# yeyupiaoling/PPASR

Hardware: AMD Instinct MI355X
Metric: audio-seconds/s (RTF^-1) Conformer-streaming fbank, batch32 per GPU, ctc_greedy (higher is better)
Workload: dtype f32; 1 GPU; configs[1]: Conformer streaming (configs/conformer.yml), fbank-80, 32 x 10 s utterances per GPU, V=4233, ctc_greedy, features resident in HBM -> token ids + scores on device; global_batch=32, frames=1000, decoder=ctc_greedy, parallelism=utterance-dp1, pipelined=False, gemm=f32

## Files before the change

ppasr_amd/csrc/capi.hip:

```cpp
#include <cxxabi.h>
#include <cstdlib>

#include "capi_internal.h"

namespace ppasr {
thread_local LaunchProf g_launch_prof;
}

static thread_local std::string g_err;
std::string& ppasr_err_slot() { return g_err; }


ppasr_status upload_pe_table(ppasr_model_s* m, BlobMap& sd, const float** pe_dev) {
  const int d = m->desc.output_size > 0 ? m->desc.output_size : kD;
  const int max_len = m->desc.max_len > 0 ? m->desc.max_len : 5000;
  m->desc.max_len = max_len;
  std::vector<float> pe((size_t)max_len * d);
  auto it = sd.find("__pe_table__");
  if (it != sd.end() && it->second.numel() == pe.size()) {
    std::memcpy(pe.data(), it->second.p, pe.size() * sizeof(float));
  } else {
    for (int i = 0; i < d / 2; ++i) {
      float div = expf((float)(2 * i) * (float)(-(std::log(10000.0) / d)));
      for (int pos = 0; pos < max_len; ++pos) {
// ... 166 lines not shown
    m->front.conv2_w = nullptr;
  } else {
    GET(mean, "encoder.global_cmvn.mean", F);
    GET(istd, "encoder.global_cmvn.istd", F);
    GET(c1w, "encoder.embed.conv.0.weight", d * 9);
    GET(c1b, "encoder.embed.conv.0.bias", d);
    const int k2 = il == 6 ? 5 : 3;
    GET(c2w, "encoder.embed.conv.2.weight", (size_t)d * d * k2 * k2);
    GET(c2b, "encoder.embed.conv.2.bias", d);
    const std::string lin = il ? "encoder.embed.linear" : "encoder.embed.out.0";
    GET(ew, lin + ".weight", (size_t)d * F2 * d);
    GET(eb, lin + ".bias", d);
    UP(vec_of(mean, F), m->front.cmvn_mean);
    UP(vec_of(istd, F), m->front.cmvn_istd);
    std::vector<float> c1(9 * d);
    for (int c = 0; c < d; ++c)
      for (int j = 0; j < 9; ++j) c1[j * d + c] = c1w[c * 9 + j];
    UP(c1, m->front.conv1_w);
    UP(vec_of(c1b, d), m->front.conv1_b);
    const int taps2 = k2 * k2;
    auto c2 = [&](int k, int n) { return c2w[((size_t)n * d + (k % d)) * taps2 + (k / d)]; };
    UP4(pack_b(taps2 * d, d, c2), m->front.conv2_w);
    m->front.conv2_wp = nullptr;
    if (il == 0 && d == kD) UP4(pack_conv2_pair(d, c2), m->front.conv2_wp);
    UP(vec_of(c2b, d), m->front.conv2_b);
    m->front.conv2_k = k2;
    m->front.conv2_s = il == 6 ? 3 : 2;
    m->front.conv3_w = nullptr;
    m->front.conv3_b = nullptr;
    if (il == 8) {
      GET(c3w, "encoder.embed.conv.4.weight", (size_t)d * d * 9);
      GET(c3b, "encoder.embed.conv.4.bias", d);
      UP4(pack_b(9 * d, d, [&](int k, int n) { return c3w[((size_t)n * d + (k % d)) * 9 + (k / d)]; }), m->front.conv3_w);
      UP(vec_of(c3b, d), m->front.conv3_b);
    }
    UP4(pack_b(F2 * d, d, [&](int k, int n) { return ew[((size_t)(k % d) * F2 + (k / d)) * d + n]; }), m->front.embed_w);
    UP(vec_of(eb, d), m->front.embed_b);
  }

  const float* pe_dev = nullptr;
  if ((st = upload_pe_table(m, sd, &pe_dev)) != PPASR_OK) return st;
  m->pe_dev = pe_dev;
  UP(std::vector<float>(d, 0.f), m->zero_vec);
  if (generic) m->gen_x.resize(desc->num_blocks);
  const int max_len = m->desc.max_len;
  m->layers.resize(desc->num_blocks);
  m->layer_ks.assign(desc->num_blocks, KS);
// ... 534 lines not shown
    PadSkip ps;
    if (skip) {
      ps.lens = lens;
      ps.Tp = Tcur;
      ps.mul = mul_cur;
      ps.slack = mul_cur == sub ? slack_full : slack_half;
    }
    return ps;
  };
  const f32x4* conv2_h3 = h->gemm_mode == PPASR_GEMM_F16X3 ? h->conv2_w_h3 : nullptr;
  const bool conv12 = h->desc.input_layer == 0 && !conv2_h3 && conv12_enabled(h) && conv12_supported(h->front, F, F2);
  const PadSkip ps_front = skip_front ? pskip(Tp, sub) : PadSkip{};
  if (!conv12) timed(0, [&] { launch_conv1(feats, h->front, y1, B, T, F, T1, F1, st, ps_front); });
  if (h->desc.input_layer == 8) {
    timed(1, [&] {
      launch_conv_stage(y1, h->front.conv2_w, h->front.conv2_b, y2, B, T1, F1, fd.T2, F2, 3, 2, st);
      launch_conv_stage(y2, h->front.conv3_w, h->front.conv3_b, y1, B, fd.T2, F2, Tp, h->F3, 3, 2, st);
    });
    timed(2, [&] { launch_embed(y1, h->front, xa, M, h->F3 * kD, sqrtf((float)kD), false, st, PadSkip{}, ffn_split_for(h, M), y2); });
  } else {
    timed(1, [&] {
      int* tile_tab = (size_t)B + 2 <= ((size_t)M + 63) / 64 * 64 ? reinterpret_cast<int*>(ws + wl.rmax) : nullptr;
      if (conv12) launch_conv12(feats, h->front, y2, B, T, F, Tp, F2, st, ps_front, tile_tab);
      else if (h->desc.input_layer == 0 && !conv2_h3 && conv2_pair_supported(h->front))
        launch_conv2_pair(y1, h->front, y2, B, T1, F1, Tp, F2, st, ps_front, tile_tab);
      else launch_conv2(y1, h->front, y2, B, T1, F1, Tp, F2, st, ps_front, tile_tab, h->desc.input_layer == 0 ? conv2_h3 : nullptr);
    });
    timed(2, [&] {
      launch_embed(y2, h->front, xa, M, F2 * kD, sqrtf((float)kD), false, st, ps_front, wide_slices_for(h, M, F2), y1,
                   conv2_h3 ? h->embed_w_h3 : nullptr);
    });
  }
  tap(xa, (size_t)M * kD);
  const int n_chunks = h->desc.linear_units / 256;
  struct BlkTab { int Ti, R; int* tab; } btabs[4];
  int n_bt = 0;
  size_t bt_off = ((size_t)B + 2 + 15) / 16 * 16;
  const bool bt_ok = skip && block_tables_enabled() && (size_t)B + 2 <= ((size_t)M + 63) / 64 * 64;
  auto with_table = [&](PadSkip p, int Tcur, int R) {
    if (!bt_ok) return p;
    for (int k = 0; k < n_bt; ++k)
      if (btabs[k].Ti == Tcur && btabs[k].R == R) { p.tab = btabs[k].tab; return p; }
    const size_t n = 1 + ((size_t)B * Tcur + R - 1) / R;
    if (n_bt == 4 || bt_off + n > 2 * (((size_t)M + 63) / 64 * 64)) return p;
    int* t = reinterpret_cast<int*>(ws + wl.rmax) + bt_off;
    launch_block_table(p, B * Tcur, R, t, st);
    btabs[n_bt++] = BlkTab{Tcur, R, t};
    bt_off += (n + 15) / 16 * 16;
// ... 767 lines not shown
```

ppasr_amd/csrc/capi_internal.h:

```cpp
#pragma once
#include <hip/hip_runtime.h>

#include <cmath>
#include <cstdio>
#include <cstring>
#include <memory>
#include <string>
#include <unordered_map>
#include <vector>

#include "../../include/ppasr_hip.h"
#include "conformer_kernels.h"
#include "launch.h"
#include "ctc_beam.h"

using namespace ppasr;

#include "squeezeformer_kernels.h"
#include "ds2_kernels.h"

std::string& ppasr_err_slot();
inline ppasr_status fail(ppasr_status s, const std::string& msg) {
  ppasr_err_slot() = msg;
  return s;
// ... 11 lines not shown
  size_t numel() const {
    size_t n = 1;
    for (int i = 0; i < ndim; ++i) n *= (size_t)shape[i];
    return n;
  }
};

template <typename Acc>
inline std::vector<float> pack_b(int K, int N, Acc w) {
  const int n_tiles = (N + 31) / 32, G = K / 8;
  std::vector<float> out((size_t)n_tiles * G * 256, 0.f);
  for (int nt = 0; nt < n_tiles; ++nt)
    for (int g = 0; g < G; ++g)
      for (int l = 0; l < 64; ++l) {
        int n = nt * 32 + (l & 31);
        if (n >= N) continue;
        float* dst = &out[(((size_t)nt * G + g) * 64 + l) * 4];
        for (int j = 0; j < 4; ++j) dst[j] = w(8 * g + 4 * (l >> 5) + j, n);
      }
  return out;
}

template <typename Acc>
inline std::vector<float> pack_conv2_pair(int d, Acc w) {
  return pack_b(24 * 128, d, [&](int k, int n) {
    const int s = k / 512, slab = (k / 128) & 3, kw = s >> 1, c = (s & 1) * 128 + (k & 127);
    const float g0 = w(kw * d + c, n), w1 = w((3 + kw) * d + c, n), g1 = w((6 + kw) * d + c, n);
    return slab == 0 ? g0 : slab == 1 ? w1 : slab == 2 ? g0 + g1 : g1;
  });
}

typedef std::unordered_map<std::string, Blob> BlobMap;

inline unsigned eff_stride_mask(const ppasr_model_desc& d) {
  if (d.model_type != PPASR_MODEL_EFFICIENT_CONFORMER) return 0u;
  if (d.stride_layer_mask != 0) return (unsigned)d.stride_layer_mask;
  return d.stride_layer_idx >= 0 ? (1u << d.stride_layer_idx) : 0u;
}
inline int eff_strides_before(const ppasr_model_desc& d, int layer) {
  return __builtin_popcount(eff_stride_mask(d) & ((1u << layer) - 1u));
}

struct ppasr_model_s {
  ppasr_model_desc desc;
  int F1, F2;
  const f32x4* gen_head_w = nullptr;
  const float* gen_head_b = nullptr;
  int gen_vpad = 0;
  int F3 = 0;
  struct Front {
    int T1, T2, Tp;
// ... 162 lines not shown
```

ppasr_amd/csrc/capi_squeezeformer.hip:

```cpp
#include "capi_internal.h"

namespace {

struct Getter {
  BlobMap& sd;
  std::string missing;
  const float* operator()(const std::string& name, size_t numel) {
    auto it = sd.find(name);
    if (it == sd.end() || it->second.numel() != numel) {
      if (missing.empty()) missing = name;
      return nullptr;
    }
    return it->second.p;
  }
};

std::vector<float> vec_of(const float* p, size_t n) { return std::vector<float>(p, p + n); }

}

#define GETW(var, name, numel)                 \
  const float* var = get(name, (size_t)(numel)); \
  if (!var) return fail(PPASR_EMISSING, "missing or mis-shaped weight: " + get.missing)
#define UP(vec, dst) \
// ... 26 lines not shown
    const bool dw_stride = !c2w;
    if (!c2w) {
      get.missing.clear();
      c2w = get("encoder.embed.dw_conv.weight", (size_t)d * 9);
    }
    if (!c2w) return fail(PPASR_EMISSING, "missing or mis-shaped weight: " + get.missing);
    GETW(c2b, "encoder.embed.dw_conv.bias", d);
    GETW(ew, "encoder.embed.input_proj.0.weight", (size_t)d * F2 * d);
    GETW(eb, "encoder.embed.input_proj.0.bias", d);
    GETW(pg, "encoder.preln.weight", d);
    GETW(pb, "encoder.preln.bias", d);
    UP(vec_of(mean, F), m->front.cmvn_mean);
    UP(vec_of(istd, F), m->front.cmvn_istd);
    std::vector<float> c1(9 * d);
    for (int c = 0; c < d; ++c)
      for (int j = 0; j < 9; ++j) c1[j * d + c] = c1w[c * 9 + j];
    UP(c1, m->front.conv1_w);
    UP(vec_of(c1b, d), m->front.conv1_b);
    auto c2 = [&](int k, int n) {
      if (dw_stride) return (k % d) == n ? c2w[(size_t)n * 9 + (k / d)] : 0.f;
      return c2w[((size_t)n * d + (k % d)) * 9 + (k / d)];
    };
    UP4(pack_b(9 * d, d, c2), m->front.conv2_w);
    if (d == kD) UP4(pack_conv2_pair(d, c2), m->front.conv2_wp);
    UP(vec_of(c2b, d), m->front.conv2_b);
    UP4(pack_b(F2 * d, d, [&](int k, int n) { return ew[((size_t)(k % d) * F2 + (k / d)) * d + n]; }), m->front.embed_w);
    UP(vec_of(eb, d), m->front.embed_b);
    UP(vec_of(pg, d), m->preln_g);
    UP(vec_of(pb, d), m->preln_b);
  }
  m->sq_layers.resize(L);
  for (int i = 0; i < L; ++i) {
    SqLayerW& W = m->sq_layers[i];
    const std::string p = "encoder.encoders." + std::to_string(i) + ".";
    auto ln = [&](const std::string& n, const float** g, const float** b) -> ppasr_status {
      const float* gw = get(p + n + ".weight", d);
      const float* gb = get(p + n + ".bias", d);
      if (!gw || !gb) return fail(PPASR_EMISSING, "missing or mis-shaped weight: " + get.missing);
      ppasr_status s1 = m->upload(vec_of(gw, d), g);
      return s1 != PPASR_OK ? s1 : m->upload(vec_of(gb, d), b);
    };
    if ((st = ln("layer_norm1", &W.ln1_g, &W.ln1_b)) != PPASR_OK) return st;
    if ((st = ln("layer_norm2", &W.ln2_g, &W.ln2_b)) != PPASR_OK) return st;
    if ((st = ln("layer_norm3", &W.ln3_g, &W.ln3_b)) != PPASR_OK) return st;
    if ((st = ln("layer_norm4", &W.ln4_g, &W.ln4_b)) != PPASR_OK) return st;
    W.cm_eps = 1e-5f;
    if (sd.find(p + "conv_module.norm._mean") != sd.end()) {
// ... 240 lines not shown
  };
  const PadSkip psF = pskip(Tp, 4), psH = pskip(Tr, 8);
  int* tile_tab = (size_t)B + 2 <= ((size_t)M + 63) / 64 * 64 ? reinterpret_cast<int*>(ws + wl.rmax) : nullptr;
  const int rowsF = h->taps ? 32 : row_block_for(h, B, Tp, 4, psF.slack, skip);
  const int rowsH = h->taps ? 32 : row_block_for(h, B, Tr, 8, psH.slack, skip);
  PadSkip psF_rb = psF, psH_rb = psH;
  if (skip && tile_tab && block_tables_enabled()) {
    const int RF = rowsF == 16 ? 16 : 32, RH = rowsH == 16 ? 16 : 32;
    const size_t nF = 1 + ((size_t)M + RF - 1) / RF, nH = 1 + ((size_t)B * Tr + RH - 1) / RH;
    const size_t o1 = ((size_t)B + 2 + 15) / 16 * 16, o2 = o1 + (nF + 15) / 16 * 16;
    if (o2 + nH <= 2 * (((size_t)M + 63) / 64 * 64)) {
      int* base = reinterpret_cast<int*>(ws + wl.rmax);
      launch_block_table(psF, M, RF, base + o1, st);
      launch_block_table(psH, B * Tr, RH, base + o2, st);
      psF_rb.tab = base + o1;
      psH_rb.tab = base + o2;
    }
  }
  const f32x4* conv2_h3 = h->gemm_mode == PPASR_GEMM_F16X3 ? h->conv2_w_h3 : nullptr;
  if (!conv2_h3 && conv12_enabled(h) && conv12_supported(h->front, F, F2)) {
    launch_conv12(feats, h->front, y2, B, T, F, Tp, F2, st, psF, tile_tab);
  } else {
    launch_conv1(feats, h->front, y1, B, T, F, T1, F1, st, psF);
    if (!conv2_h3 && conv2_pair_supported(h->front)) launch_conv2_pair(y1, h->front, y2, B, T1, F1, Tp, F2, st, psF, tile_tab);
    else launch_conv2(y1, h->front, y2, B, T1, F1, Tp, F2, st, psF, tile_tab, conv2_h3);
  }
  launch_embed(y2, h->front, xa, M, F2 * kD, sqrtf((float)kD), true, st,
               (rowsF != 16 && ffn_split_for(h, M) == 1) ? psF_rb : psF, ffn_split_for(h, M), y1,
               conv2_h3 ? h->embed_w_h3 : nullptr);
  launch_ln_rows(xa, h->preln_g, h->preln_b, M, st, psF);
  tap(xa, (size_t)M * kD);
  float* x = xa;
  float* other = xb;
  bool reduced = false;
  bool have_qkv = false;
  for (int i = 0; i < L; ++i) {
    const SqLayerW& W = h->sq_layers[i];
    if (i == h->desc.reduce_idx) {
      HIP_TRY(hipMemcpyAsync(xs, x, (size_t)M * kD * sizeof(float), hipMemcpyDeviceToDevice, st));
      launch_sq_reduce(x, other, qkv, h->sq_reduce, W.wqkv, W.bqkv, lens, B, Tp, Tr, st, psH);
      std::swap(x, other);
      reduced = true;
      have_qkv = true;
    }
    if (i == h->desc.recover_idx && reduced) {
      launch_sq_recover(x, xs, other, qkv, h->sq_wrec, h->sq_brec, W.wqkv, W.bqkv, B, Tp, Tr, st, psF);
      std::swap(x, other);
// ... 87 lines not shown
```

ppasr_amd/csrc/conformer_kernels.h:

```cpp
#pragma once
#include <hip/hip_runtime.h>
#include <stdint.h>

#include "rowblock.h"

namespace ppasr {

struct LayerW {
  const float *ln_mac_g, *ln_mac_b, *ln_mha_g, *ln_mha_b, *ln_conv_g, *ln_conv_b;
  const float *ln_ff_g, *ln_ff_b, *ln_fin_g, *ln_fin_b, *ln_cm_g, *ln_cm_b;
  float cm_eps;
  const f32x4 *ffm_w1, *ffm_w2, *ff_w1, *ff_w2, *wqkv, *wo, *pw1, *pw2;
  const float *ffm_b1, *ffm_b2, *ff_b1, *ff_b2, *bqkv, *bo, *pw1_b, *pw2_b;
  const float *dw_w;
  const float *dw_b;
  const float *glu_pad;
  const float *pos_u, *pos_v;
  const float *ptab;
};

struct FrontW {
  const float *cmvn_mean, *cmvn_istd;
  const float *conv1_w, *conv1_b;
  const f32x4 *conv2_w;
// ... 38 lines not shown
  int q_frames, kv_frames;
  int group;
  const SessDesc* sess;
  long long sess_stride;
  int pad_skip;
  const float* vt = nullptr;
  int vt_stride = 0;
  int dm = 256;
};
struct VtOut {
  float* vt = nullptr;
  int stride = 0;
  int k_h3 = 0;
};

constexpr size_t kLdsExclusive = 82 * 1024;
size_t ragged_lds(size_t lds, const PadSkip& ps, int n_blocks);

bool launch_attention_t(const AttnArgs& a, int B, int H, hipStream_t st);
hipError_t configure_attention_kernels();

void launch_block_table(const PadSkip& ps, int M, int R, int* tab, hipStream_t st);

bool conv2_pair_supported(const FrontW& fw);
bool conv12_supported(const FrontW& fw, int F, int F2);
void launch_conv12(const float* feats, const FrontW& fw, float* y2, int B, int T, int F, int Tp, int F2, hipStream_t st,
                   const PadSkip& ps_frames, int* tile_scratch);
void launch_conv2_pair(const float* y1, const FrontW& fw, float* y2, int B, int T1, int F1, int Tp, int F2, hipStream_t st,
                       const PadSkip& ps_frames, int* tile_scratch);
hipError_t configure_front_fused_kernels();

void launch_ffn_qkv_16(const float* x_in, float* x1, float* qkv, const LayerW& w, int M, int n_chunks, hipStream_t st,
                       const PadSkip& ps);
void launch_out_glu_16(const float* ctx, const float* x1, float* x2, float* g, const LayerW& w, const int64_t* lens, int M,
                       int Tp, int mask_mul, hipStream_t st, const PadSkip& ps);
void launch_out_glu_split_16(const float* ctx, const float* x1, float* x2, float* g, float* xhat, const LayerW& w,
                             const int64_t* lens, int M, int Tp, int mask_mul, hipStream_t st, const PadSkip& ps,
                             float* hist = nullptr, int lo = 0);
void launch_shift_caches(float* kc, float* vc, long long layer_stride, int D, int n_layers, int from_full, int keep_full,
                         int from_half, int keep_half, unsigned long long half_mask, hipStream_t st);
void launch_oproj_ln_16(const float* ctx, const float* x1, float* x2_sink, float* xhat_out, const LayerW& w, int M,
                        hipStream_t st, const PadSkip& ps = PadSkip{});
void launch_pw1_glu_cols_16(const float* x, float* g, const LayerW& w, int M, hipStream_t st, float* hist = nullptr, int lo = 0,
                            const float* hist_scale = nullptr, const float* hist_bias = nullptr, const PadSkip& ps = PadSkip{},
                            const int64_t* lens = nullptr, int Tp = 1, int mask_mul = 1);
bool conv_ffn_16_supported(int ksize, int Tp);
void launch_conv_ffn_16(const float* g, const float* x2, float* x_out, const LayerW& w, const int64_t* lens, int M, int Tp,
                        int n_chunks, int ksize, int mask_mul, const LayerW* next, float* x1_next, float* qkv_next,
                        hipStream_t st, bool causal, const PadSkip& ps);
void launch_ffn_qkv_w16(const float* x_in, float* x1, float* qkv, const LayerW& w, int M, int n_chunks, hipStream_t st,
                        const PadSkip& ps, VtOut vt);
// ... 119 lines not shown
```

ppasr_amd/csrc/front_fused.hip:

```cpp
#include "conformer_kernels.h"
#include "launch.h"

namespace ppasr {

template <int MT, bool FROM_Y1>
__device__ __forceinline__ void conv2_pair_body(const float* __restrict__ src, const FrontW& fw, float* __restrict__ out,
                                                int T, int F, int Tp, int F2, int M, int m0, const PadSkip& ps,
                                                const int* __restrict__ tile_tab) {
  constexpr int BP = 32 * MT, KC = 128, LD = KC + 4, G = KC / 8, NL = 2 * MT, N_STAGES = 6, N_CHUNKS = 4 * N_STAGES;
  constexpr int SLOT = 2 * BP * LD;
  const int P = (Tp + 1) >> 1;
  int r0 = m0 + blockIdx.x * BP, Mlim = M;
  if (tile_tab) {
    const int t = blockIdx.x, nb = tile_tab[0];
    const int* pre = tile_tab + 1;
    if (t >= pre[nb]) return;
    int lo = 0, hi = nb;
    while (hi - lo > 1) {
      const int mid = (lo + hi) >> 1;
      if (pre[mid] <= t) lo = mid;
      else hi = mid;
    }
    const int S = ps.Tp * ps.unit;
    r0 = lo * S + (t - pre[lo]) * BP;
    Mlim = min(M, (lo + 1) * S);
  } else if (pad_block_skippable(ps, r0, BP, M)) {
    return;
  }
  extern __shared__ __attribute__((aligned(16))) float smem[];
  float* const slot0 = smem;
  float* const slot1 = smem + SLOT;
  const int tid = threadIdx.x, lane = lane_id(), wave = wave_id();
  constexpr int tile_stride = N_CHUNKS * G * 64;
  const f32x4* wbase = fw.conv2_wp + (size_t)wave * tile_stride;
  BRing<1> ring;
  ring_prime(ring, wbase, 0);
  const int c4 = tid & 31, rbase = tid >> 5;
  const int bp0 = r0 / F2;
  float* xs = smem + 2 * SLOT;
  uint32_t pb[MT];
  int yrow[FROM_Y1 ? NL : 1], yp4[FROM_Y1 ? NL : 1], yf[FROM_Y1 ? NL : 1];
  if constexpr (!FROM_Y1) {
    const int nbp = (min(r0 + BP, Mlim) - 1) / F2 - bp0 + 1;
    for (int idx = tid; idx < nbp * 11 * F; idx += kThreads) {
      const int q = idx / F, f = idx - q * F;
      const int bpl = q / 11, fr = q - 11 * bpl;
      const int bp = bp0 + bpl, b = bp / P, p = bp - b * P;
      const int t = min(8 * p + fr, T - 1);
      xs[idx] = (src[((size_t)b * T + t) * F + f] - fw.cmvn_mean[f]) * fw.cmvn_istd[f];
    }
#pragma unroll
    for (int i = 0; i < NL; ++i) {
      const int m = r0 + rbase + 16 * i;
      const int bp = m / F2, f2 = m - bp * F2;
      const uint32_t v = m < Mlim ? (uint32_t)((bp - bp0) * 11 * F + 4 * f2) : 0xffffu;
      pb[i >> 1] = (i & 1) ? (pb[i >> 1] | (v << 16)) : v;
    }
  } else {
#pragma unroll
    for (int i = 0; i < NL; ++i) {
      const int m = r0 + rbase + 16 * i;
      const int bp = m / F2, f2 = m - bp * F2, b = bp / P, p = bp - b * P;
      yrow[i] = b * T + 4 * p;
      yp4[i] = 4 * p;
      yf[i] = m < Mlim ? 2 * f2 : -1;
    }
  }
  auto pbase = [&](int i) { return (int)((i & 1) ? (pb[i >> 1] >> 16) : (pb[i >> 1] & 0xffffu)); };
  const int lds_off0 = rbase * LD + 4 * c4;
  f32x4 wv[FROM_Y1 ? 1 : 9], bv;
  float xv[9];
  f32x4 yv;
  auto load_w = [&](int s) {
    if constexpr (!FROM_Y1) {
      const int c = (s & 1) * 128 + 4 * c4;
#pragma unroll
      for (int j = 0; j < 9; ++j) wv[j] = *reinterpret_cast<const f32x4*>(fw.conv1_w + j * 256 + c);
      bv = *reinterpret_cast<const f32x4*>(fw.conv1_b + c);
    }
  };
  auto y1_read = [&](int i, int s, int j) {
    const int kw = s >> 1;
    if constexpr (!FROM_Y1) {
      const int o = pbase(i);
      const float* p = xs + (o == 0xffff ? 0 : o) + 2 * j * F + 2 * kw;
#pragma unroll
      for (int ii = 0; ii < 3; ++ii)
#pragma unroll
        for (int jj = 0; jj < 3; ++jj) xv[ii * 3 + jj] = p[ii * F + jj];
    } else {
      yv = f32x4{0.f, 0.f, 0.f, 0.f};
      if (yf[i] >= 0 && yp4[i] + j < T)
        yv = *reinterpret_cast<const f32x4*>(src + ((size_t)(yrow[i] + j) * F + yf[i] + kw) * 256 + (s & 1) * 128 + 4 * c4);
    }
  };
  auto y1_value = [&](int i) {
    if constexpr (!FROM_Y1) {
      f32x4 a = {0.f, 0.f, 0.f, 0.f};
#pragma unroll
      for (int j = 0; j < 9; ++j)
#pragma unroll
        for (int e = 0; e < 4; ++e) a[e] = fmaf(wv[j][e], xv[j], a[e]);
      a += bv;
#pragma unroll
      for (int e = 0; e < 4; ++e) a[e] = pbase(i) != 0xffff ? fmaxf(a[e], 0.f) : 0.f;
      return a;
    } else {
      return yv;
    }
  };
  auto put = [&](float* buf, int row16, const f32x4& v) {
    *reinterpret_cast<f32x4*>(buf + lds_off0 + row16 * 16 * LD) = v;
  };
  f32x4 d1c[NL], d0;
  auto side_d01 = [&](int s, int g) {
    const int e = g >> 1, i = e >> 1;
    if (e >= 2 * NL) return;
    if ((g & 1) == 0) {
      y1_read(i, s, (e & 1) ? 2 : 0);
    } else if ((e & 1) == 0) {
      d0 = y1_value(i);
    } else {
      d1c[i] = y1_value(i);
      put(slot0, i, d0 - d1c[i]);
    }
  };
  auto side_o = [&](int s, int g) {
    const int e = g >> 1, hi = e >= NL, i = e - (hi ? NL : 0);
    if (e >= 2 * NL) return;
    if ((g & 1) == 0) y1_read(i, s, hi ? 3 : 1);
    else put(slot1, hi ? NL + i : i, y1_value(i));
  };
  auto side_d1 = [&](int g) {
    if (g < NL) put(slot0, g, d1c[g]);
  };
  auto side_d21 = [&](int s, int g) {
    const int e = g >> 1;
    if (e >= NL) return;
    if ((g & 1) == 0) y1_read(e, s, 4);
    else put(slot1, e, y1_value(e) - d1c[e]);
  };
  load_w(0);
  __syncthreads();
#pragma unroll
  for (int g = 0; g < 2 * G; ++g) {
    side_d01(0, g);
    __builtin_amdgcn_sched_barrier(0);
  }
  __syncthreads();
  f32x16 accA[MT][1], accB[MT][1], accS[MT][1];
  acc_zero(accA);
  acc_zero(accB);
  acc_zero(accS);
  for (int s = 0; s < N_STAGES; ++s) {
    const f32x4* seg = wbase + (size_t)(4 * s) * G * 64;
    {
      auto side = [&](int g) { side_o(s, g); };
      rb_gemm<MT, 1, G, kPF, decltype(side)>(slot0, LD, seg, 0, seg + G * 64, 0, ring, accA, side);
    }
    __syncthreads();
    {
      auto side = [&](int g) { side_d1(g); };
      rb_gemm<MT, 1, G, kPF, decltype(side)>(slot1, LD, seg + G * 64, 0, seg + G * 64, 0, ring, accA, side);
      rb_gemm<MT, 1, G>(slot1 + BP * LD, LD, seg + G * 64, 0, seg + 2 * G * 64, 0, ring, accB);
    }
    __syncthreads();
    {
      auto side = [&](int g) { side_d21(s, g); };
      rb_gemm<MT, 1, G, kPF, decltype(side)>(slot0, LD, seg + 2 * G * 64, 0, seg + 3 * G * 64, 0, ring, accS, side);
    }
    __syncthreads();
    if (s + 1 < N_STAGES) {
      load_w(s + 1);
      auto side = [&](int g) { side_d01(s + 1, g); };
      rb_gemm<MT, 1, G, kPF, decltype(side)>(slot1, LD, seg + 3 * G * 64, 0, seg + 4 * G * 64, 0, ring, accB, side);
    } else {
      rb_gemm<MT, 1, G>(slot1, LD, seg + 3 * G * 64, 0, nullptr, 0, ring, accB);
    }
    __syncthreads();
  }
  const int col = wave * 32 + (lane & 31);
  const float b2 = fw.conv2_b[col];
#pragma unroll
  for (int mt = 0; mt < MT; ++mt)
#pragma unroll
    for (int r = 0; r < 16; ++r) {
      const int m = r0 + mt * 32 + acc_row(r, lane);
      if (m >= Mlim) continue;
      const int bp = m / F2, f2 = m - bp * F2, b = bp / P, t0 = 2 * (bp - b * P);
      const float s = accS[mt][0][r];
      float* o = out + ((size_t)(b * Tp + t0) * F2 + f2) * 256 + col;
      o[0] = fmaxf(accA[mt][0][r] + s + b2, 0.f);
      if (t0 + 1 < Tp) o[(size_t)F2 * 256] = fmaxf(s + accB[mt][0][r] + b2, 0.f);
    }
}

template <int MT>
__global__ __launch_bounds__(kThreads) void k_conv12(const float* __restrict__ feats, FrontW fw, float* __restrict__ out,
                                                     int T, int F, int Tp, int F2, int M, int m0, PadSkip ps,
                                                     const int* __restrict__ tile_tab) {
  conv2_pair_body<MT, false>(feats, fw, out, T, F, Tp, F2, M, m0, ps, tile_tab);
}
template <int MT>
__global__ __launch_bounds__(kThreads) void k_conv2_pair(const float* __restrict__ y1, FrontW fw, float* __restrict__ out,
                                                         int T1, int F1, int Tp, int F2, int M, int m0, PadSkip ps,
                                                         const int* __restrict__ tile_tab) {
  conv2_pair_body<MT, true>(y1, fw, out, T1, F1, Tp, F2, M, m0, ps, tile_tab);
}

static size_t pair_lds(int mt, bool fused, int F, int F2) {
  const int bp = 32 * mt, nbp = (bp - 1) / F2 + 2;
  return ((size_t)2 * 2 * bp * 132 + (fused ? (size_t)nbp * 11 * F : 0)) * sizeof(float);
}
bool conv2_pair_supported(const FrontW& fw) { return fw.conv2_wp && fw.conv2_k == 3 && fw.conv2_s == 2; }
bool conv12_supported(const FrontW& fw, int F, int F2) {
  return conv2_pair_supported(fw) && F2 >= 1 && pair_lds(1, true, F, F2) <= 160 * 1024 &&
         (size_t)((31 / F2) + 2) * 11 * F < 0xffff;
}

void launch_tile_prefix(const PadSkip& ps, int B, int BM, int* tab, hipStream_t st);

static void launch_pair(bool fused, const float* src, const FrontW& fw, float* y2, int B, int T, int F, int Tp, int F2,
                        hipStream_t st, const PadSkip& ps_frames, int* tile_scratch) {
  const int P = (Tp + 1) / 2;
  PadSkip ps = ps_frames;
  ps.Tp = P;
  ps.mul = 2 * ps_frames.mul;
  ps.slack = (ps_frames.slack + 1) / 2;
  ps.unit = F2;
  const int M = B * P * F2;
  const int* no_tab = nullptr;
#define PAIR(MTA, GRID, M0, TAB)                                                                                        \
  do {                                                                                                                 \
    if (fused)                                                                                                         \
      PPASR_LAUNCH(k_conv12<MTA>, dim3(GRID), dim3(kThreads), pair_lds(MTA, true, F, F2), st, src, fw, y2, T, F, Tp, F2, \
                   M, M0, ps, TAB);                                                                                    \
    else                                                                                                               \
      PPASR_LAUNCH(k_conv2_pair<MTA>, dim3(GRID), dim3(kThreads), pair_lds(MTA, false, F, F2), st, src, fw, y2, T, F,   \
                   Tp, F2, M, M0, ps, TAB);                                                                            \
  } while (0)
  if (ps.lens && tile_scratch) {
    launch_tile_prefix(ps, B, 32, tile_scratch, st);
    PAIR(1, B * ((P * F2 + 31) / 32), 0, (const int*)tile_scratch);
    return;
  }
  PAIR(1, (M + 31) / 32, 0, no_tab);
#undef PAIR
}

void launch_conv12(const float* feats, const FrontW& fw, float* y2, int B, int T, int F, int Tp, int F2, hipStream_t st,
                   const PadSkip& ps_frames, int* tile_scratch) {
  launch_pair(true, feats, fw, y2, B, T, F, Tp, F2, st, ps_frames, tile_scratch);
}
void launch_conv2_pair(const float* y1, const FrontW& fw, float* y2, int B, int T1, int F1, int Tp, int F2, hipStream_t st,
                       const PadSkip& ps_frames, int* tile_scratch) {
  launch_pair(false, y1, fw, y2, B, T1, F1, Tp, F2, st, ps_frames, tile_scratch);
}

hipError_t configure_front_fused_kernels() {
  hipError_t e;
#define SET_LDS(fn)                                                                                              \
  e = hipFuncSetAttribute(reinterpret_cast<const void*>(fn), hipFuncAttributeMaxDynamicSharedMemorySize, 160 * 1024); \
  if (e != hipSuccess) return e;
  SET_LDS(k_conv12<1>);
  SET_LDS(k_conv2_pair<1>);
#undef SET_LDS
  return hipSuccess;
}

}
```

Baseline: 55790 audio-s/s.

## Replace pair-wise conv2 Winograd-style kernel with 2x2 quad output tiling

The fused conv1+conv2 front-end kernel now computes a 2x2 block of conv2 outputs (two time steps by two frequency bins) per row instead of a pair along time. It uses a minimal-filtering decomposition with 25 input-difference chunks, combined weight slabs packed on the host, and accumulator folding. The aim is to cut the number of MFMA GEMM passes per output for the 3x3 stride-2 convolution. In exchange it needs more accumulators and extra LDS for y2 staging and conv1 weights, and the chunk schedule is considerably more complex.

```diff
diff --git a/ppasr_amd/csrc/capi.hip b/ppasr_amd/csrc/capi.hip
--- a/ppasr_amd/csrc/capi.hip
+++ b/ppasr_amd/csrc/capi.hip
@@ -212,7 +212,7 @@
     auto c2 = [&](int k, int n) { return c2w[((size_t)n * d + (k % d)) * taps2 + (k / d)]; };
     UP4(pack_b(taps2 * d, d, c2), m->front.conv2_w);
     m->front.conv2_wp = nullptr;
-    if (il == 0 && d == kD) UP4(pack_conv2_pair(d, c2), m->front.conv2_wp);
+    if (il == 0 && d == kD) UP4(pack_conv2_quad(d, c2), m->front.conv2_wp);
     UP(vec_of(c2b, d), m->front.conv2_b);
     m->front.conv2_k = k2;
     m->front.conv2_s = il == 6 ? 3 : 2;
@@ -793,8 +793,8 @@
     timed(1, [&] {
       int* tile_tab = (size_t)B + 2 <= ((size_t)M + 63) / 64 * 64 ? reinterpret_cast<int*>(ws + wl.rmax) : nullptr;
       if (conv12) launch_conv12(feats, h->front, y2, B, T, F, Tp, F2, st, ps_front, tile_tab);
-      else if (h->desc.input_layer == 0 && !conv2_h3 && conv2_pair_supported(h->front))
-        launch_conv2_pair(y1, h->front, y2, B, T1, F1, Tp, F2, st, ps_front, tile_tab);
+      else if (h->desc.input_layer == 0 && !conv2_h3 && conv2_quad_supported(h->front))
+        launch_conv2_quad(y1, h->front, y2, B, T1, F1, Tp, F2, st, ps_front, tile_tab);
       else launch_conv2(y1, h->front, y2, B, T1, F1, Tp, F2, st, ps_front, tile_tab, h->desc.input_layer == 0 ? conv2_h3 : nullptr);
     });
     timed(2, [&] {
diff --git a/ppasr_amd/csrc/capi_internal.h b/ppasr_amd/csrc/capi_internal.h
--- a/ppasr_amd/csrc/capi_internal.h
+++ b/ppasr_amd/csrc/capi_internal.h
@@ -57,11 +57,16 @@
 }
 
 template <typename Acc>
-inline std::vector<float> pack_conv2_pair(int d, Acc w) {
-  return pack_b(24 * 128, d, [&](int k, int n) {
-    const int s = k / 512, slab = (k / 128) & 3, kw = s >> 1, c = (s & 1) * 128 + (k & 127);
-    const float g0 = w(kw * d + c, n), w1 = w((3 + kw) * d + c, n), g1 = w((6 + kw) * d + c, n);
-    return slab == 0 ? g0 : slab == 1 ? w1 : slab == 2 ? g0 + g1 : g1;
+inline std::vector<float> pack_conv2_quad(int d, Acc w) {
+  static const int taps[4][2] = {{0, -1}, {1, -1}, {0, 2}, {2, -1}};
+  return pack_b(32 * 128, d, [&](int k, int n) {
+    const int h = k / 2048, slab = (k / 128) & 15, c = h * 128 + (k & 127);
+    const int* th = taps[slab >> 2];
+    const int* tw = taps[slab & 3];
+    double v = 0.0;
+    for (int a = 0; a < 2 && th[a] >= 0; ++a)
+      for (int e = 0; e < 2 && tw[e] >= 0; ++e) v += (double)w((th[a] * 3 + tw[e]) * d + c, n);
+    return (float)v;
   });
 }
 
diff --git a/ppasr_amd/csrc/capi_squeezeformer.hip b/ppasr_amd/csrc/capi_squeezeformer.hip
--- a/ppasr_amd/csrc/capi_squeezeformer.hip
+++ b/ppasr_amd/csrc/capi_squeezeformer.hip
@@ -72,7 +72,7 @@
       return c2w[((size_t)n * d + (k % d)) * 9 + (k / d)];
     };
     UP4(pack_b(9 * d, d, c2), m->front.conv2_w);
-    if (d == kD) UP4(pack_conv2_pair(d, c2), m->front.conv2_wp);
+    if (d == kD) UP4(pack_conv2_quad(d, c2), m->front.conv2_wp);
     UP(vec_of(c2b, d), m->front.conv2_b);
     UP4(pack_b(F2 * d, d, [&](int k, int n) { return ew[((size_t)(k % d) * F2 + (k / d)) * d + n]; }), m->front.embed_w);
     UP(vec_of(eb, d), m->front.embed_b);
@@ -359,7 +359,7 @@
     launch_conv12(feats, h->front, y2, B, T, F, Tp, F2, st, psF, tile_tab);
   } else {
     launch_conv1(feats, h->front, y1, B, T, F, T1, F1, st, psF);
-    if (!conv2_h3 && conv2_pair_supported(h->front)) launch_conv2_pair(y1, h->front, y2, B, T1, F1, Tp, F2, st, psF, tile_tab);
+    if (!conv2_h3 && conv2_quad_supported(h->front)) launch_conv2_quad(y1, h->front, y2, B, T1, F1, Tp, F2, st, psF, tile_tab);
     else launch_conv2(y1, h->front, y2, B, T1, F1, Tp, F2, st, psF, tile_tab, conv2_h3);
   }
   launch_embed(y2, h->front, xa, M, F2 * kD, sqrtf((float)kD), true, st,
diff --git a/ppasr_amd/csrc/conformer_kernels.h b/ppasr_amd/csrc/conformer_kernels.h
--- a/ppasr_amd/csrc/conformer_kernels.h
+++ b/ppasr_amd/csrc/conformer_kernels.h
@@ -84,11 +84,11 @@
 
 void launch_block_table(const PadSkip& ps, int M, int R, int* tab, hipStream_t st);
 
-bool conv2_pair_supported(const FrontW& fw);
+bool conv2_quad_supported(const FrontW& fw);
 bool conv12_supported(const FrontW& fw, int F, int F2);
 void launch_conv12(const float* feats, const FrontW& fw, float* y2, int B, int T, int F, int Tp, int F2, hipStream_t st,
                    const PadSkip& ps_frames, int* tile_scratch);
-void launch_conv2_pair(const float* y1, const FrontW& fw, float* y2, int B, int T1, int F1, int Tp, int F2, hipStream_t st,
+void launch_conv2_quad(const float* y1, const FrontW& fw, float* y2, int B, int T1, int F1, int Tp, int F2, hipStream_t st,
                        const PadSkip& ps_frames, int* tile_scratch);
 hipError_t configure_front_fused_kernels();
 
diff --git a/ppasr_amd/csrc/front_fused.hip b/ppasr_amd/csrc/front_fused.hip
--- a/ppasr_amd/csrc/front_fused.hip
+++ b/ppasr_amd/csrc/front_fused.hip
@@ -1,15 +1,48 @@
+#include <utility>
+
 #include "conformer_kernels.h"
 #include "launch.h"
 
 namespace ppasr {
 
-template <int MT, bool FROM_Y1>
-__device__ __forceinline__ void conv2_pair_body(const float* __restrict__ src, const FrontW& fw, float* __restrict__ out,
+namespace {
+constexpr int kGroupRow[5] = {2, 0, 1, 4, 3};
+constexpr int kTapCol[5] = {2, 0, 1, 4, 3};
+constexpr int kFactor[5] = {2, 0, 1, 3, 1};
+constexpr int quad_slab(int t) { return 4 * kFactor[t / 5] + kFactor[t % 5]; }
+constexpr int quad_target(int t) {
+  const int g = t / 5, k = t % 5;
+  if (g == 0) return k == 0 ? 4 : k <= 2 ? 5 : 4;
+  const int a = (g == 1 || g == 2) ? 0 : 2;
+  return k == 0 ? (a == 0 ? 5 : 4) : k <= 2 ? a : a + 1;
+}
+constexpr int quad_fold_src(int t) {
+  return t == 1 || t == 5 || t == 21 || t == 23 ? 4 : t == 3 || t == 11 || t == 13 ? 5 : -1;
+}
+constexpr int quad_fold_mask(int t) {
+  return t == 1 ? 0xf : t == 3 ? 0x5 : t == 5 ? 0xa : t == 11 ? 0x2 : t == 13 ? 0x1 : t == 21 ? 0x8 : t == 23 ? 0x4 : 0;
+}
+constexpr bool quad_fold_clear(int t) { return t == 1 || t == 3 || t == 5 || t == 13 || t == 23; }
+static_assert(quad_target(0) == 4 && quad_target(2) == 5 && quad_target(10) == 5 && quad_target(12) == 0 &&
+                  quad_target(14) == 1 && quad_target(20) == 4 && quad_target(22) == 2 && quad_target(24) == 3,
+              "chunk targets");
+
+template <typename Fn, int... I>
+__device__ __forceinline__ void static_for(std::integer_sequence<int, I...>, Fn&& fn) {
+  (fn(std::integral_constant<int, I>{}), ...);
+}
+
+__host__ __device__ inline int quad_xs_stride(int F, int Q) { return F > 8 * Q + 3 ? F : 8 * Q + 3; }
+}
+
+template <bool FROM_Y1>
+__device__ __forceinline__ void conv2_quad_body(const float* __restrict__ src, const FrontW& fw, float* __restrict__ out,
                                                 int T, int F, int Tp, int F2, int M, int m0, const PadSkip& ps,
                                                 const int* __restrict__ tile_tab) {
-  constexpr int BP = 32 * MT, KC = 128, LD = KC + 4, G = KC / 8, NL = 2 * MT, N_STAGES = 6, N_CHUNKS = 4 * N_STAGES;
-  constexpr int SLOT = 2 * BP * LD;
+  constexpr int BP = 32, KC = 128, LD = KC + 4, G = KC / 8, NL = 2, N_CHUNKS = 25;
+  constexpr int SLOT = BP * LD;
   const int P = (Tp + 1) >> 1;
+  const int Q = (F2 + 1) >> 1;
   int r0 = m0 + blockIdx.x * BP, Mlim = M;
   if (tile_tab) {
     const int t = blockIdx.x, nb = tile_tab[0];
@@ -30,231 +63,236 @@
   extern __shared__ __attribute__((aligned(16))) float smem[];
   float* const slot0 = smem;
   float* const slot1 = smem + SLOT;
+  f32x4* const y2s = reinterpret_cast<f32x4*>(smem + 2 * SLOT);
+  float* const w1s = smem + 2 * SLOT + 5 * NL * 4 * kThreads;
+  float* const xs = w1s + 10 * 256;
   const int tid = threadIdx.x, lane = lane_id(), wave = wave_id();
-  constexpr int tile_stride = N_CHUNKS * G * 64;
+  constexpr int tile_stride = 2 * 16 * G * 64;
   const f32x4* wbase = fw.conv2_wp + (size_t)wave * tile_stride;
+  auto seg = [&](int h, int slab) { return wbase + (size_t)(16 * h + slab) * G * 64; };
   BRing<1> ring;
-  ring_prime(ring, wbase, 0);
+  ring_prime(ring, seg(0, quad_slab(0)), 0);
   const int c4 = tid & 31, rbase = tid >> 5;
-  const int bp0 = r0 / F2;
-  float* xs = smem + 2 * SLOT;
-  uint32_t pb[MT];
-  int yrow[FROM_Y1 ? NL : 1], yp4[FROM_Y1 ? NL : 1], yf[FROM_Y1 ? NL : 1];
+  const int bp0 = r0 / Q;
+  const int FX = quad_xs_stride(F, Q);
+  uint32_t pb = 0;
+  int yrow[FROM_Y1 ? NL : 1], yp4[FROM_Y1 ? NL : 1], yq4[FROM_Y1 ? NL : 1];
   if constexpr (!FROM_Y1) {
-    const int nbp = (min(r0 + BP, Mlim) - 1) / F2 - bp0 + 1;
-    for (int idx = tid; idx < nbp * 11 * F; idx += kThreads) {
-      const int q = idx / F, f = idx - q * F;
-      const int bpl = q / 11, fr = q - 11 * bpl;
+    for (int idx = tid; idx < 10 * 256; idx += kThreads) w1s[idx] = idx < 9 * 256 ? fw.conv1_w[idx] : fw.conv1_b[idx - 9 * 256];
+    const int nbp = (min(r0 + BP, Mlim) - 1) / Q - bp0 + 1;
+    for (int idx = tid; idx < nbp * 11 * FX; idx += kThreads) {
+      const int fr_row = idx / FX, f = idx - fr_row * FX;
+      const int bpl = fr_row / 11, fr = fr_row - 11 * bpl;
       const int bp = bp0 + bpl, b = bp / P, p = bp - b * P;
       const int t = min(8 * p + fr, T - 1);
-      xs[idx] = (src[((size_t)b * T + t) * F + f] - fw.cmvn_mean[f]) * fw.cmvn_istd[f];
+      xs[idx] = f < F ? (src[((size_t)b * T + t) * F + f] - fw.cmvn_mean[f]) * fw.cmvn_istd[f] : 0.f;
     }
 #pragma unroll
     for (int i = 0; i < NL; ++i) {
       const int m = r0 + rbase + 16 * i;
-      const int bp = m / F2, f2 = m - bp * F2;
-      const uint32_t v = m < Mlim ? (uint32_t)((bp - bp0) * 11 * F + 4 * f2) : 0xffffu;
-      pb[i >> 1] = (i & 1) ? (pb[i >> 1] | (v << 16)) : v;
+      const int bp = m / Q, q = m - bp * Q;
+      const uint32_t v = m < Mlim ? (uint32_t)((bp - bp0) * 11 * FX + 8 * q) : 0xffffu;
+      pb |= v << (16 * i);
     }
   } else {
 #pragma unroll
     for (int i = 0; i < NL; ++i) {
       const int m = r0 + rbase + 16 * i;
-      const int bp = m / F2, f2 = m - bp * F2, b = bp / P, p = bp - b * P;
+      const int bp = m / Q, q = m - bp * Q, b = bp / P, p = bp - b * P;
       yrow[i] = b * T + 4 * p;
       yp4[i] = 4 * p;
-      yf[i] = m < Mlim ? 2 * f2 : -1;
-    }
-  }
-  auto pbase = [&](int i) { return (int)((i & 1) ? (pb[i >> 1] >> 16) : (pb[i >> 1] & 0xffffu)); };
+      yq4[i] = m < Mlim ? 4 * q : -1;
+    }
+  }
+  auto pbase = [&](int i) { return (int)((pb >> (16 * i)) & 0xffffu); };
   const int lds_off0 = rbase * LD + 4 * c4;
-  f32x4 wv[FROM_Y1 ? 1 : 9], bv;
   float xv[9];
-  f32x4 yv;
-  auto load_w = [&](int s) {
+  f32x4 wv[3], bv, ya, yv;
+  auto y1_step = [&](int i, int h, int r, int c, int step) {
+    const int cc = h * 128 + 4 * c4;
     if constexpr (!FROM_Y1) {
-      const int c = (s & 1) * 128 + 4 * c4;
-#pragma unroll
-      for (int j = 0; j < 9; ++j) wv[j] = *reinterpret_cast<const f32x4*>(fw.conv1_w + j * 256 + c);
-      bv = *reinterpret_cast<const f32x4*>(fw.conv1_b + c);
+      if (step == 0) {
+        const int o = pbase(i);
+        const float* p = xs + (o == 0xffff ? 0 : o) + 2 * r * FX + 2 * c;
+#pragma unroll
+        for (int ii = 0; ii < 3; ++ii)
+#pragma unroll
+          for (int jj = 0; jj < 3; ++jj) xv[ii * 3 + jj] = p[ii * FX + jj];
+        ya = f32x4{0.f, 0.f, 0.f, 0.f};
+      } else {
+#pragma unroll
+        for (int j = 3 * (step - 1); j < 3 * step; ++j)
+#pragma unroll
+          for (int e = 0; e < 4; ++e) ya[e] = fmaf(wv[j % 3][e], xv[j], ya[e]);
+        if (step == 3) {
+          ya += bv;
+#pragma unroll
+          for (int e = 0; e < 4; ++e) ya[e] = pbase(i) != 0xffff ? fmaxf(ya[e], 0.f) : 0.f;
+        }
+      }
+      if (step < 3) {
+#pragma unroll
+        for (int j = 0; j < 3; ++j) wv[j] = *reinterpret_cast<const f32x4*>(w1s + (3 * step + j) * 256 + cc);
+        if (step == 2) bv = *reinterpret_cast<const f32x4*>(w1s + 9 * 256 + cc);
+      }
+    } else {
+      if (step == 0) {
+        yv = f32x4{0.f, 0.f, 0.f, 0.f};
+        if (yq4[i] >= 0 && yp4[i] + r < T && yq4[i] + c < F)
+          yv = *reinterpret_cast<const f32x4*>(src + ((size_t)(yrow[i] + r) * F + yq4[i] + c) * 256 + cc);
+      } else if (step == 3) {
+        ya = yv;
+      }
     }
   };
-  auto y1_read = [&](int i, int s, int j) {
-    const int kw = s >> 1;
+  auto put = [&](float* buf, int i, const f32x4& v) { *reinterpret_cast<f32x4*>(buf + lds_off0 + i * 16 * LD) = v; };
+  auto y2row = [&](int c, int i) -> f32x4& { return y2s[(c * NL + i) * kThreads + tid]; };
+  f32x4 z2[NL];
+  auto build = [&](auto nc, int g, int h, float* buf) {
+    constexpr int n = decltype(nc)::value, grp = n / 5, k = n % 5, r = kGroupRow[grp], c = kTapCol[k];
+    const int i = g >> 2, step = g & 3;
+    y1_step(i, h, r, c, step);
+    if (step != 3) return;
+    f32x4 v = ya;
+    if constexpr (grp == 0) y2row(c, i) = ya;
+    if constexpr (grp == 1 || grp == 3) v = ya - y2row(c, i);
+    if constexpr (k == 0) {
+      z2[i] = v;
+      put(buf, i, v);
+    } else if constexpr (k == 1 || k == 3) {
+      put(buf, i, v - z2[i]);
+    } else {
+      put(buf, i, v);
+    }
+  };
+  f32x16 acc[6][1][1];
+#pragma unroll
+  for (int a = 0; a < 6; ++a) acc_zero(acc[a]);
+  auto fold = [&](auto tc, int g) {
+    constexpr int t = decltype(tc)::value, fs = quad_fold_src(t), mask = quad_fold_mask(t);
+    if constexpr (fs >= 0) {
+      const int j = g - 4 * NL;
+      int seen = 0;
+#pragma unroll
+      for (int o = 0; o < 4; ++o) {
+        if (!((mask >> o) & 1)) continue;
+        if (seen++ == j) {
+#pragma unroll
+          for (int e = 0; e < 16; ++e) asm volatile("v_add_f32 %0, %0, %1" : "+v"(acc[o][0][0][e]) : "v"(acc[fs][0][0][e]));
+        }
+      }
+      if (quad_fold_clear(t) && j == 4) acc_zero(acc[fs]);
+    }
+  };
+  __syncthreads();
+#pragma unroll
+  for (int g = 0; g < 4 * NL; ++g) {
+    build(std::integral_constant<int, 0>{}, g, 0, slot0);
+    __builtin_amdgcn_sched_barrier(0);
+  }
+  __syncthreads();
+  for (int h = 0; h < 2; ++h) {
+    asm volatile("" : "+s"(wbase));
     if constexpr (!FROM_Y1) {
-      const int o = pbase(i);
-      const float* p = xs + (o == 0xffff ? 0 : o) + 2 * j * F + 2 * kw;
-#pragma unroll
-      for (int ii = 0; ii < 3; ++ii)
-#pragma unroll
-        for (int jj = 0; jj < 3; ++jj) xv[ii * 3 + jj] = p[ii * F + jj];
+      asm volatile("" : "+v"(pb));
     } else {
-      yv = f32x4{0.f, 0.f, 0.f, 0.f};
-      if (yf[i] >= 0 && yp4[i] + j < T)
-        yv = *reinterpret_cast<const f32x4*>(src + ((size_t)(yrow[i] + j) * F + yf[i] + kw) * 256 + (s & 1) * 128 + 4 * c4);
-    }
-  };
-  auto y1_value = [&](int i) {
-    if constexpr (!FROM_Y1) {
-      f32x4 a = {0.f, 0.f, 0.f, 0.f};
-#pragma unroll
-      for (int j = 0; j < 9; ++j)
-#pragma unroll
-        for (int e = 0; e < 4; ++e) a[e] = fmaf(wv[j][e], xv[j], a[e]);
-      a += bv;
-#pragma unroll
-      for (int e = 0; e < 4; ++e) a[e] = pbase(i) != 0xffff ? fmaxf(a[e], 0.f) : 0.f;
-      return a;
-    } else {
-      return yv;
-    }
-  };
-  auto put = [&](float* buf, int row16, const f32x4& v) {
-    *reinterpret_cast<f32x4*>(buf + lds_off0 + row16 * 16 * LD) = v;
-  };
-  f32x4 d1c[NL], d0;
-  auto side_d01 = [&](int s, int g) {
-    const int e = g >> 1, i = e >> 1;
-    if (e >= 2 * NL) return;
-    if ((g & 1) == 0) {
-      y1_read(i, s, (e & 1) ? 2 : 0);
-    } else if ((e & 1) == 0) {
-      d0 = y1_value(i);
-    } else {
-      d1c[i] = y1_value(i);
-      put(slot0, i, d0 - d1c[i]);
-    }
-  };
-  auto side_o = [&](int s, int g) {
-    const int e = g >> 1, hi = e >= NL, i = e - (hi ? NL : 0);
-    if (e >= 2 * NL) return;
-    if ((g & 1) == 0) y1_read(i, s, hi ? 3 : 1);
-    else put(slot1, hi ? NL + i : i, y1_value(i));
-  };
-  auto side_d1 = [&](int g) {
-    if (g < NL) put(slot0, g, d1c[g]);
-  };
-  auto side_d21 = [&](int s, int g) {
-    const int e = g >> 1;
-    if (e >= NL) return;
-    if ((g & 1) == 0) y1_read(e, s, 4);
-    else put(slot1, e, y1_value(e) - d1c[e]);
-  };
-  load_w(0);
-  __syncthreads();
-#pragma unroll
-  for (int g = 0; g < 2 * G; ++g) {
-    side_d01(0, g);
-    __builtin_amdgcn_sched_barrier(0);
-  }
-  __syncthreads();
-  f32x16 accA[MT][1], accB[MT][1], accS[MT][1];
-  acc_zero(accA);
-  acc_zero(accB);
-  acc_zero(accS);
-  for (int s = 0; s < N_STAGES; ++s) {
-    const f32x4* seg = wbase + (size_t)(4 * s) * G * 64;
-    {
-      auto side = [&](int g) { side_o(s, g); };
-      rb_gemm<MT, 1, G, kPF, decltype(side)>(slot0, LD, seg, 0, seg + G * 64, 0, ring, accA, side);
-    }
-    __syncthreads();
-    {
-      auto side = [&](int g) { side_d1(g); };
-      rb_gemm<MT, 1, G, kPF, decltype(side)>(slot1, LD, seg + G * 64, 0, seg + G * 64, 0, ring, accA, side);
-      rb_gemm<MT, 1, G>(slot1 + BP * LD, LD, seg + G * 64, 0, seg + 2 * G * 64, 0, ring, accB);
-    }
-    __syncthreads();
-    {
-      auto side = [&](int g) { side_d21(s, g); };
-      rb_gemm<MT, 1, G, kPF, decltype(side)>(slot0, LD, seg + 2 * G * 64, 0, seg + 3 * G * 64, 0, ring, accS, side);
-    }
-    __syncthreads();
-    if (s + 1 < N_STAGES) {
-      load_w(s + 1);
-      auto side = [&](int g) { side_d01(s + 1, g); };
-      rb_gemm<MT, 1, G, kPF, decltype(side)>(slot1, LD, seg + 3 * G * 64, 0, seg + 4 * G * 64, 0, ring, accB, side);
-    } else {
-      rb_gemm<MT, 1, G>(slot1, LD, seg + 3 * G * 64, 0, nullptr, 0, ring, accB);
-    }
-    __syncthreads();
+#pragma unroll
+      for (int i = 0; i < NL; ++i) asm volatile("" : "+v"(yrow[i]), "+v"(yp4[i]), "+v"(yq4[i]));
+    }
+    static_for(std::make_integer_sequence<int, N_CHUNKS>{}, [&](auto tc) {
+      constexpr int t = decltype(tc)::value;
+      float* const cur = ((t + h) & 1) ? slot1 : slot0;
+      float* const nxb = ((t + h) & 1) ? slot0 : slot1;
+      const f32x4* nseg = t + 1 < N_CHUNKS ? seg(h, quad_slab(t + 1)) : (h == 0 ? seg(1, quad_slab(0)) : nullptr);
+      auto side = [&](int g) {
+        if (g < 4 * NL) {
+          if constexpr (t + 1 < N_CHUNKS) build(std::integral_constant<int, t + 1>{}, g, h, nxb);
+          else if (h == 0) build(std::integral_constant<int, 0>{}, g, 1, nxb);
+        } else {
+          fold(tc, g);
+        }
+      };
+      rb_gemm<1, 1, G, kPF, decltype(side)>(cur, LD, seg(h, quad_slab(t)), 0, nseg, 0, ring, acc[quad_target(t)], side);
+      __syncthreads();
+    });
   }
   const int col = wave * 32 + (lane & 31);
   const float b2 = fw.conv2_b[col];
 #pragma unroll
-  for (int mt = 0; mt < MT; ++mt)
-#pragma unroll
-    for (int r = 0; r < 16; ++r) {
-      const int m = r0 + mt * 32 + acc_row(r, lane);
-      if (m >= Mlim) continue;
-      const int bp = m / F2, f2 = m - bp * F2, b = bp / P, t0 = 2 * (bp - b * P);
-      const float s = accS[mt][0][r];
-      float* o = out + ((size_t)(b * Tp + t0) * F2 + f2) * 256 + col;
-      o[0] = fmaxf(accA[mt][0][r] + s + b2, 0.f);
-      if (t0 + 1 < Tp) o[(size_t)F2 * 256] = fmaxf(s + accB[mt][0][r] + b2, 0.f);
-    }
-}
-
-template <int MT>
+  for (int r = 0; r < 16; ++r) {
+    const int m = r0 + acc_row(r, lane);
+    if (m >= Mlim) continue;
+    const int bp = m / Q, q = m - bp * Q, b = bp / P, t0 = 2 * (bp - b * P), f0 = 2 * q;
+    float* o = out + ((size_t)(b * Tp + t0) * F2 + f0) * 256 + col;
+    const bool f1 = f0 + 1 < F2, t1 = t0 + 1 < Tp;
+    o[0] = fmaxf(acc[0][0][0][r] + b2, 0.f);
+    if (f1) o[256] = fmaxf(acc[1][0][0][r] + b2, 0.f);
+    if (t1) o[(size_t)F2 * 256] = fmaxf(acc[2][0][0][r] + b2, 0.f);
+    if (t1 && f1) o[(size_t)F2 * 256 + 256] = fmaxf(acc[3][0][0][r] + b2, 0.f);
+  }
+}
+
 __global__ __launch_bounds__(kThreads) void k_conv12(const float* __restrict__ feats, FrontW fw, float* __restrict__ out,
                                                      int T, int F, int Tp, int F2, int M, int m0, PadSkip ps,
                                                      const int* __restrict__ tile_tab) {
-  conv2_pair_body<MT, false>(feats, fw, out, T, F, Tp, F2, M, m0, ps, tile_tab);
-}
-template <int MT>
+  conv2_quad_body<false>(feats, fw, out, T, F, Tp, F2, M, m0, ps, tile_tab);
+}
 __global__ __launch_bounds__(kThreads) void k_conv2_pair(const float* __restrict__ y1, FrontW fw, float* __restrict__ out,
                                                          int T1, int F1, int Tp, int F2, int M, int m0, PadSkip ps,
                                                          const int* __restrict__ tile_tab) {
-  conv2_pair_body<MT, true>(y1, fw, out, T1, F1, Tp, F2, M, m0, ps, tile_tab);
-}
-
-static size_t pair_lds(int mt, bool fused, int F, int F2) {
-  const int bp = 32 * mt, nbp = (bp - 1) / F2 + 2;
-  return ((size_t)2 * 2 * bp * 132 + (fused ? (size_t)nbp * 11 * F : 0)) * sizeof(float);
-}
-bool conv2_pair_supported(const FrontW& fw) { return fw.conv2_wp && fw.conv2_k == 3 && fw.conv2_s == 2; }
+  conv2_quad_body<true>(y1, fw, out, T1, F1, Tp, F2, M, m0, ps, tile_tab);
+}
+
+static int quad_tile_pairs(int Q) { return 31 / Q + 2; }
+static size_t quad_lds(bool fused, int F, int F2) {
+  const int Q = (F2 + 1) / 2;
+  return ((size_t)2 * 32 * 132 + (size_t)5 * 2 * 4 * 512 + (fused ? (size_t)10 * 256 + (size_t)quad_tile_pairs(Q) * 11 * quad_xs_stride(F, Q) : 0)) *
+         sizeof(float);
+}
+bool conv2_quad_supported(const FrontW& fw) { return fw.conv2_wp && fw.conv2_k == 3 && fw.conv2_s == 2; }
 bool conv12_supported(const FrontW& fw, int F, int F2) {
-  return conv2_pair_supported(fw) && F2 >= 1 && pair_lds(1, true, F, F2) <= 160 * 1024 &&
-         (size_t)((31 / F2) + 2) * 11 * F < 0xffff;
+  const int Q = (F2 + 1) / 2;
+  return conv2_quad_supported(fw) && F2 >= 1 && quad_lds(true, F, F2) <= 160 * 1024 &&
+         (size_t)quad_tile_pairs(Q) * 11 * quad_xs_stride(F, Q) < 0xffff;
 }
 
 void launch_tile_prefix(const PadSkip& ps, int B, int BM, int* tab, hipStream_t st);
 
-static void launch_pair(bool fused, const float* src, const FrontW& fw, float* y2, int B, int T, int F, int Tp, int F2,
+static void launch_quad(bool fused, const float* src, const FrontW& fw, float* y2, int B, int T, int F, int Tp, int F2,
                         hipStream_t st, const PadSkip& ps_frames, int* tile_scratch) {
-  const int P = (Tp + 1) / 2;
+  const int P = (Tp + 1) / 2, Q = (F2 + 1) / 2;
   PadSkip ps = ps_frames;
   ps.Tp = P;
   ps.mul = 2 * ps_frames.mul;
   ps.slack = (ps_frames.slack + 1) / 2;
-  ps.unit = F2;
-  const int M = B * P * F2;
+  ps.unit = Q;
+  const int M = B * P * Q;
   const int* no_tab = nullptr;
-#define PAIR(MTA, GRID, M0, TAB)                                                                                        \
+#define QUAD(GRID, TAB)                                                                                                  \
   do {                                                                                                                 \
     if (fused)                                                                                                         \
-      PPASR_LAUNCH(k_conv12<MTA>, dim3(GRID), dim3(kThreads), pair_lds(MTA, true, F, F2), st, src, fw, y2, T, F, Tp, F2, \
-                   M, M0, ps, TAB);                                                                                    \
+      PPASR_LAUNCH(k_conv12, dim3(GRID), dim3(kThreads), quad_lds(true, F, F2), st, src, fw, y2, T, F, Tp, F2, M, 0, ps, \
+                   TAB);                                                                                               \
     else                                                                                                               \
-      PPASR_LAUNCH(k_conv2_pair<MTA>, dim3(GRID), dim3(kThreads), pair_lds(MTA, false, F, F2), st, src, fw, y2, T, F,   \
-                   Tp, F2, M, M0, ps, TAB);                                                                            \
+      PPASR_LAUNCH(k_conv2_pair, dim3(GRID), dim3(kThreads), quad_lds(false, F, F2), st, src, fw, y2, T, F, Tp, F2, M, 0, \
+                   ps, TAB);                                                                                           \
   } while (0)
   if (ps.lens && tile_scratch) {
     launch_tile_prefix(ps, B, 32, tile_scratch, st);
-    PAIR(1, B * ((P * F2 + 31) / 32), 0, (const int*)tile_scratch);
+    QUAD(B * ((P * Q + 31) / 32), (const int*)tile_scratch);
     return;
   }
-  PAIR(1, (M + 31) / 32, 0, no_tab);
-#undef PAIR
+  QUAD((M + 31) / 32, no_tab);
+#undef QUAD
 }
 
 void launch_conv12(const float* feats, const FrontW& fw, float* y2, int B, int T, int F, int Tp, int F2, hipStream_t st,
                    const PadSkip& ps_frames, int* tile_scratch) {
-  launch_pair(true, feats, fw, y2, B, T, F, Tp, F2, st, ps_frames, tile_scratch);
-}
-void launch_conv2_pair(const float* y1, const FrontW& fw, float* y2, int B, int T1, int F1, int Tp, int F2, hipStream_t st,
+  launch_quad(true, feats, fw, y2, B, T, F, Tp, F2, st, ps_frames, tile_scratch);
+}
+void launch_conv2_quad(const float* y1, const FrontW& fw, float* y2, int B, int T1, int F1, int Tp, int F2, hipStream_t st,
                        const PadSkip& ps_frames, int* tile_scratch) {
-  launch_pair(false, y1, fw, y2, B, T1, F1, Tp, F2, st, ps_frames, tile_scratch);
+  launch_quad(false, y1, fw, y2, B, T1, F1, Tp, F2, st, ps_frames, tile_scratch);
 }
 
 hipError_t configure_front_fused_kernels() {
@@ -262,8 +300,8 @@
 #define SET_LDS(fn)                                                                                              \
   e = hipFuncSetAttribute(reinterpret_cast<const void*>(fn), hipFuncAttributeMaxDynamicSharedMemorySize, 160 * 1024); \
   if (e != hipSuccess) return e;
-  SET_LDS(k_conv12<1>);
-  SET_LDS(k_conv2_pair<1>);
+  SET_LDS(k_conv12);
+  SET_LDS(k_conv2_pair);
 #undef SET_LDS
   return hipSuccess;
 }
```

After: 57870 audio-s/s, median of 6. 3.7% higher.
